# jwliao1209/DiffMusic

Hardware: AMD Instinct MI355X
Metric: denoising steps/sec (10 s clip, 200-step DPS) (higher is better)
Workload: dtype f16; 1 GPU; MusicLDM + DPS music_inpainting, 10 s @16 kHz, 200-step schedule, batch 8 per GPU (BASELINE.json configs[1]); global_batch=8, clips_per_gpu=8, lanes=1, parallelism=clip-sharded x1 (RCCL world size 1, no per-step collective), finite=True, nan_steps=0, settle_steps=10, cached_reference_transform=True, launched_by=single process

## Files before the change

### diffmusic_amd/_lib.py

```python
import ctypes as C
import os

_HERE = os.path.dirname(os.path.abspath(__file__))
LIB_PATH = os.environ.get("DMX_LIB_PATH") or os.path.join(_HERE, "lib", "libdiffmusic_hip.so")
MAX_STAGES = 8


class HifiGanConfig(C.Structure):
    _fields_ = [("model_in_dim", C.c_int), ("upsample_initial_channel", C.c_int), ("num_upsamples", C.c_int),
                ("upsample_rates", C.c_int * MAX_STAGES), ("upsample_kernel_sizes", C.c_int * MAX_STAGES),
                ("num_kernels", C.c_int), ("resblock_kernel_sizes", C.c_int * MAX_STAGES),
                ("num_dilations", C.c_int), ("resblock_dilation_sizes", C.c_int * (MAX_STAGES * MAX_STAGES)),
                ("leaky_relu_slope", C.c_float)]


class VaeConfig(C.Structure):
    _fields_ = [("latent_channels", C.c_int), ("out_channels", C.c_int), ("num_blocks", C.c_int),
                ("block_out_channels", C.c_int * MAX_STAGES), ("layers_per_block", C.c_int),
                ("norm_num_groups", C.c_int), ("eps", C.c_float)]


class UNetConfig(C.Structure):
    _fields_ = [("in_channels", C.c_int), ("out_channels", C.c_int), ("num_blocks", C.c_int),
                ("block_out_channels", C.c_int * MAX_STAGES), ("layers_per_block", C.c_int),
# ... 65 lines not shown
    "dmx_vae_encode_fwd": (C.c_int, [C.c_void_p, C.c_void_p, C.c_float, C.c_void_p, C.c_int, C.c_int, C.c_int, C.c_void_p, C.c_size_t,
                                     C.c_void_p]),
    "dmx_latent_init": (C.c_int, [C.c_void_p] * 6 + [C.c_int] * 3 + [C.c_float] * 3 + [C.c_void_p]),
    "dmx_conv2d_raw": (C.c_int, [C.c_void_p] * 4 + [C.c_int] * 9 + [C.c_void_p]),
    "dmx_unet_workspace_bytes": (C.c_size_t, [C.c_void_p, C.c_int, C.c_int, C.c_int]),
    "dmx_unet_fwd": (C.c_int, [C.c_void_p, C.c_void_p, C.c_void_p, C.c_void_p, C.c_void_p, C.c_int, C.c_int, C.c_int,
                               C.c_void_p, C.c_size_t, C.c_void_p]),
    "dmx_unet_fwd_ctx": (C.c_int, [C.c_void_p] * 5 + [C.c_int, C.c_void_p, C.c_int, C.c_void_p, C.c_void_p, C.c_int, C.c_int, C.c_int,
                                   C.c_void_p, C.c_size_t, C.c_void_p]),
    "dmx_unet_workspace_bytes_ctx": (C.c_size_t, [C.c_void_p, C.c_int, C.c_int, C.c_int, C.c_int, C.c_int]),
    "dmx_htsat_create": (C.c_void_p, [C.POINTER(HtsatConfig)]),
    "dmx_htsat_feature_dims": (C.c_int, [C.c_void_p, C.POINTER(C.c_int), C.POINTER(C.c_int)]),
    "dmx_htsat_workspace_bytes": (C.c_size_t, [C.c_void_p, C.c_int, C.c_int]),
    "dmx_htsat_fwd": (C.c_int, [C.c_void_p, C.c_void_p, C.c_int, C.c_int, C.c_void_p, C.c_int, C.c_void_p, C.c_size_t, C.c_void_p]),
    "dmx_htsat_bwd": (C.c_int, [C.c_void_p, C.c_void_p, C.c_void_p, C.c_void_p, C.c_void_p]),
    "dmx_htsat_tape_raw": (C.c_size_t, [C.c_void_p, C.c_int, C.c_int, C.c_int, C.c_void_p, C.c_size_t, C.c_void_p]),
    "dmx_gram_fwd": (C.c_int, [C.c_void_p, C.c_void_p, C.c_int, C.c_int, C.c_int, C.c_void_p]),
    "dmx_gram_bwd": (C.c_int, [C.c_void_p, C.c_void_p, C.c_void_p, C.c_int, C.c_int, C.c_int, C.c_void_p]),
    "dmx_gemm_raw": (C.c_int, [C.c_void_p, C.c_size_t, C.c_void_p]),
    "dmx_prof_begin": (None, []),
    "dmx_prof_end": (C.c_int, [C.POINTER(C.c_double), C.POINTER(C.c_double)]),
    "dmx_flash_attn_raw": (C.c_int, [C.c_void_p, C.c_void_p, C.c_void_p, C.c_void_p, C.c_void_p] + [C.c_int] * 6 + [C.c_float, C.c_void_p]),
    "dmx_flash_attn_ld_raw": (C.c_int, [C.c_void_p] * 5 + [C.c_int] * 8 + [C.c_float, C.POINTER(C.c_int), C.c_void_p]),
    "dmx_softmax_raw": (C.c_int, [C.c_void_p] * 3 + [C.c_longlong, C.c_int, C.c_longlong, C.c_longlong, C.c_int, C.c_void_p]),
    "dmx_softmax_act_raw": (C.c_int, [C.c_void_p] * 3 + [C.c_longlong, C.c_int, C.c_longlong, C.c_int, C.c_void_p]),
    "dmx_transpose_raw": (C.c_int, [C.c_void_p, C.c_void_p, C.c_int, C.c_int, C.c_longlong, C.c_longlong, C.c_int, C.c_int] + [C.c_longlong] * 4
                          + [C.c_void_p]),
    "dmx_rowdot_raw": (C.c_int, [C.c_void_p] * 3 + [C.c_longlong, C.c_int, C.c_longlong, C.c_longlong, C.c_void_p]),
    "dmx_layernorm_raw": (C.c_int, [C.c_void_p] * 4 + [C.c_int, C.c_int, C.c_float, C.c_void_p]),
    "dmx_geglu_raw": (C.c_int, [C.c_void_p, C.c_void_p, C.c_longlong, C.c_int, C.c_void_p]),
    "dmx_gemm_splitk_workspace": (C.c_int, [C.c_void_p, C.c_size_t]),
    "dmx_conv_pair_raw": (C.c_int, [C.c_void_p, C.c_void_p, C.c_size_t, C.c_void_p]),
    "dmx_conv_pair_group_raw": (C.c_int, [C.c_int, C.c_void_p, C.c_void_p, C.c_size_t, C.c_void_p]),
    "dmx_groupnorm_scratch_floats": (C.c_size_t, [C.c_int, C.c_int, C.c_int]),
    "dmx_groupnorm_raw": (C.c_int, [C.c_void_p] * 8 + [C.c_int] * 4 + [C.c_float, C.c_int, C.c_void_p]),
    "dmx_groupnorm_part_floats": (C.c_size_t, [C.c_int, C.c_int, C.c_int]),
    "dmx_groupnorm_parts_raw": (C.c_int, [C.c_void_p] * 7 + [C.c_int] * 4 + [C.c_float, C.c_int, C.c_int, C.c_void_p, C.c_void_p, C.c_void_p]),
    "dmx_gemm_last_tile_rows_raw": (C.c_int, []),
    "dmx_groupnorm_bwd_raw": (C.c_int, [C.c_void_p] * 10 + [C.c_int] * 6 + [C.c_void_p, C.c_void_p, C.c_void_p]),
    "dmx_prof_dominant": (C.c_int, [C.POINTER(C.c_double)] * 3),
    "dmx_audio_create": (C.c_void_p, [C.c_int, C.c_int, C.c_int, C.c_int, C.c_void_p]),
    "dmx_audio_destroy": (None, [C.c_void_p]),
    "dmx_audio_num_frames": (C.c_int, [C.c_void_p, C.c_int]),
    "dmx_audio_num_bins": (C.c_int, [C.c_void_p]),
    "dmx_audio_state_bytes": (C.c_size_t, [C.c_void_p, C.c_int, C.c_int]),
    "dmx_audio_transform_fwd": (C.c_int, [C.c_void_p, C.c_void_p, C.c_longlong, C.c_void_p, C.c_void_p, C.c_int, C.c_int, C.c_int,
                                          C.c_int, C.c_float, C.c_float, C.c_void_p]),
    "dmx_audio_transform_bwd": (C.c_int, [C.c_void_p, C.c_void_p, C.c_void_p, C.c_longlong, C.c_void_p, C.c_int, C.c_int, C.c_int,
                                          C.c_int, C.c_float, C.c_float, C.c_int, C.c_void_p]),
    "dmx_audio_is_fused": (C.c_int, [C.c_void_p, C.c_int]),
    "dmx_audio_guidance_fwd": (C.c_int, [C.c_void_p, C.c_void_p, C.c_longlong, C.c_void_p, C.c_void_p, C.c_longlong, C.c_void_p, C.c_void_p,
                                         C.c_int, C.c_int, C.c_int, C.c_int, C.c_float, C.c_float, C.c_void_p]),
    "dmx_audio_guidance_bwd": (C.c_int, [C.c_void_p, C.c_void_p, C.c_longlong, C.c_void_p, C.c_void_p, C.c_longlong, C.c_float, C.c_void_p,
                                         C.c_void_p, C.c_longlong, C.c_int, C.c_void_p, C.c_int, C.c_int, C.c_int, C.c_int, C.c_float, C.c_float,
                                         C.c_void_p]),
    "dmx_audio_guidance_fwd_ex": (C.c_int, [C.c_void_p, C.c_void_p, C.c_longlong, C.c_void_p, C.c_void_p, C.c_longlong, C.c_void_p, C.c_void_p,
                                            C.c_int, C.c_int, C.c_int, C.c_int, C.c_float, C.c_float, C.c_void_p, C.c_longlong, C.c_void_p,
                                            C.c_float, C.c_void_p]),
    "dmx_audio_guidance_bwd_ex": (C.c_int, [C.c_void_p, C.c_void_p, C.c_longlong, C.c_void_p, C.c_void_p, C.c_longlong, C.c_float, C.c_void_p,
                                            C.c_void_p, C.c_longlong, C.c_int, C.c_void_p, C.c_int, C.c_int, C.c_int, C.c_int, C.c_float, C.c_float,
                                            C.c_void_p, C.c_longlong, C.c_void_p, C.c_float, C.c_void_p]),
    "dmx_audio_guidance_fwd_shaped": (C.c_int, [C.c_void_p, C.c_void_p, C.c_longlong, C.c_void_p, C.c_void_p, C.c_longlong, C.c_void_p, C.c_void_p,
                                                C.c_int, C.c_int, C.c_int, C.c_int, C.c_float, C.c_float, C.c_void_p, C.c_longlong, C.c_void_p,
                                                C.c_float, C.c_void_p, C.c_void_p]),
    "dmx_audio_guidance_bwd_shaped": (C.c_int, [C.c_void_p, C.c_void_p, C.c_longlong, C.c_void_p, C.c_void_p, C.c_longlong, C.c_float, C.c_void_p,
                                                C.c_void_p, C.c_longlong, C.c_int, C.c_void_p, C.c_int, C.c_int, C.c_int, C.c_int, C.c_float, C.c_float,
# ... 86 lines not shown
```

### diffmusic_amd/csrc/capi.hip

```cpp
#include "conv_pair.h"
#include "models.h"

#define M_IMPL(m) ((m) ? (m)->impl : nullptr)
#define ST(s) ((hipStream_t)(s))

extern "C" {

int dmx_abi_version(void) { return DMX_ABI_VERSION; }
int dmx_act_dtype(void) { return DMX_ACT_DTYPE; }

dmx_model* dmx_hifigan_create(const dmx_hifigan_config* cfg) {
  if (!cfg || cfg->num_upsamples > DMX_MAX_STAGES || cfg->num_kernels > DMX_MAX_STAGES || cfg->num_dilations > DMX_MAX_STAGES) {
    dmx_set_error("bad hifigan config");
    return nullptr;
  }
  return new dmx_model{dmx_make_hifigan(cfg)};
}
dmx_model* dmx_vae_decoder_create(const dmx_vae_config* cfg) {
  if (!cfg || cfg->num_blocks > DMX_MAX_STAGES) { dmx_set_error("bad vae config"); return nullptr; }
  Model* m = dmx_make_vae(cfg);
  return m ? new dmx_model{m} : nullptr;
}
dmx_model* dmx_unet_create(const dmx_unet_config* cfg) {
  if (!cfg || cfg->num_blocks > DMX_MAX_STAGES) { dmx_set_error("bad unet config"); return nullptr; }
// ... 138 lines not shown
}

size_t dmx_unet_workspace_bytes(dmx_model* m, int batch, int h, int w) { return dmx_unet_ws_impl(m->impl, batch, h, w, 0, 0); }
size_t dmx_unet_workspace_bytes_ctx(dmx_model* m, int batch, int h, int w, int n0, int n1) { return dmx_unet_ws_impl(m->impl, batch, h, w, n0, n1); }
int dmx_unet_fwd(dmx_model* m, const float* x, const float* t, const float* class_labels, float* eps, int batch, int h, int w,
                 void* ws, size_t ws_bytes, void* stream) {
  int rc = check(m, DMX_MODEL_UNET);
  if (rc) return rc;
  if (!ws) { dmx_set_error("null workspace"); return DMX_ERR_WORKSPACE; }
  return dmx_unet_fwd_impl(m->impl, x, t, class_labels, eps, batch, h, w, ws, ws_bytes, ST(stream), nullptr, 0, nullptr, 0, nullptr);
}
int dmx_unet_fwd_ctx(dmx_model* m, const float* x, const float* t, const float* class_labels, const float* ctx0, int n0,
                     const float* ctx1, int n1, const float* bias1, float* eps, int batch, int h, int w, void* ws, size_t ws_bytes,
                     void* stream) {
  int rc = check(m, DMX_MODEL_UNET);
  if (rc) return rc;
  if (!ws) { dmx_set_error("null workspace"); return DMX_ERR_WORKSPACE; }
  return dmx_unet_fwd_impl(m->impl, x, t, class_labels, eps, batch, h, w, ws, ws_bytes, ST(stream), ctx0, n0, ctx1, n1, bias1);
}

static thread_local int g_raw_gn_rows = 0;
int dmx_gemm_raw(const void* desc, size_t desc_bytes, void* stream) {
  if (desc_bytes != sizeof(GemmDesc)) { dmx_set_error("GemmDesc size mismatch: %zu vs %zu", desc_bytes, sizeof(GemmDesc)); return DMX_ERR_SHAPE; }
  return dmx_gemm_launch(*reinterpret_cast<const GemmDesc*>(desc), ST(stream), &g_raw_gn_rows);
}
int dmx_gemm_last_tile_rows_raw(void) { return g_raw_gn_rows; }

int dmx_conv_pair_raw(const void* desc_a, const void* desc_b, size_t desc_bytes, void* stream) {
  if (desc_bytes != sizeof(GemmDesc)) { dmx_set_error("GemmDesc size mismatch: %zu vs %zu", desc_bytes, sizeof(GemmDesc)); return DMX_ERR_SHAPE; }
  const GemmDesc* a = reinterpret_cast<const GemmDesc*>(desc_a);
  const GemmDesc& b = *reinterpret_cast<const GemmDesc*>(desc_b);
  if (!dmx_conv_pair_eligible(a, b)) { dmx_set_error("shape not handled by the fused convolution-pair kernel"); return DMX_ERR_SHAPE; }
  return dmx_conv_pair_launch(a, b, ST(stream));
}

int dmx_conv_pair_group_raw(int n, const void* descs_a, const void* descs_b, size_t desc_bytes, void* stream) {
  if (desc_bytes != sizeof(GemmDesc)) { dmx_set_error("GemmDesc size mismatch: %zu vs %zu", desc_bytes, sizeof(GemmDesc)); return DMX_ERR_SHAPE; }
  if (n < 1 || n > 3) { dmx_set_error("conv pair group: 1..3 problems"); return DMX_ERR_SHAPE; }
  const GemmDesc* a = reinterpret_cast<const GemmDesc*>(descs_a);
  const GemmDesc* b = reinterpret_cast<const GemmDesc*>(descs_b);
  const GemmDesc* pa[3]; const GemmDesc* pb[3];
  for (int j = 0; j < n; ++j) { pa[j] = a + j; pb[j] = b + j; }
  const int rc = dmx_conv_pair_group_launch(n, pa, pb, ST(stream));
  if (rc == DMX_ERR_SHAPE) dmx_set_error("shape not handled by the fused convolution-pair kernel");
  return rc;
}

int dmx_flash_attn_raw(const void* q, const void* k, const void* v, void* o, const float* colbias, int B, int Nq, int Nk, int ldv, int C,
                       int heads, float scale, void* stream) {
  const int rc = dmx_flash_attn_fwd((const act_t*)q, (const act_t*)k, (const act_t*)v, (act_t*)o, colbias, B, Nq, Nk, C, heads, scale,
                                    ST(stream), 0, 0, ldv);
  if (rc == DMX_ERR_SHAPE) dmx_set_error("flash attention: unsupported head_dim / strides");
  return rc;
}

int dmx_flash_attn_ld_raw(const void* q, const void* k, const void* v, void* o, const float* colbias, int B, int Nq, int Nk, int ldq, int ldk,
                          int ldv, int C, int heads, float scale, int* qt_out, void* stream) {
  if (qt_out) *qt_out = 0;
  if (B < 1 || heads < 1 || C < heads || C % heads) { dmx_set_error("flash attention: C %d is not heads %d x head_dim", C, heads); return DMX_ERR_SHAPE; }
  const int rc = dmx_flash_attn_fwd((const act_t*)q, (const act_t*)k, (const act_t*)v, (act_t*)o, colbias, B, Nq, Nk, C, heads, scale,
                                    ST(stream), ldq, ldk, ldv, qt_out);
  if (rc == DMX_ERR_SHAPE)
    dmx_set_error("flash attention: head_dim %d (multiples of 8 up to 96), Nq %d, Nk %d (>= 1) or row strides %d / %d / %d (multiples of 8) unsupported",
                  C / heads, Nq, Nk, ldq, ldk, ldv);
  return rc;
}
// ... 85 lines not shown
```

### diffmusic_amd/csrc/conv_pair.hip

```cpp
#include "gemm_epilogue.h"
#include "conv_pair.h"

namespace {

constexpr int PAIR_HALO = 50;
constexpr int PAIR_ROWS = 256;
constexpr unsigned PAIR_OOB = 0x80000000u;

struct PairParams {
  GemmDesc a, b;
  int T, nb, BMo;
  int loA, hiA, loB, hiB;
  int off0A, dA, off0B, dB;
  int single;
  int r_from_slab;
  int a_tape_bits_only;
  int skip_q0, skip_n;
  int z0, z1;
};

#ifdef DMX_PAIR_STAMPS
__device__ unsigned long long g_pair_stamps[4096 * 8];
#define DMX_STAMP(i) do { stamp_v[i] = wall_clock64(); } while (0)
#else
#define DMX_STAMP(i) do { } while (0)
#endif

template <int C>
struct PairCfg {
  static constexpr int PITCH = 2 * C + 32;
  static constexpr int CPR = C / 8;
  static constexpr int WN = C > 64 ? C / 64 : 1;
  static constexpr int NW = 4 * WN;
  static constexpr int NT = NW * 64;
  static constexpr int FN = C / 16 / WN;
  static constexpr int SLAB_ROWS = PAIR_ROWS + PAIR_HALO;
  static constexpr int SLAB_BYTES = SLAB_ROWS * PITCH;
  static constexpr int TILE = C * 128;
  static constexpr int NS = C == 128 ? 4 : 3;
  static constexpr int PER = TILE / 1024 / NW;
  static constexpr int SLAB_IT = (SLAB_ROWS * CPR + NT - 1) / NT;
  static constexpr int BITS_IT = PAIR_ROWS * CPR / NT;
  static constexpr int BITS_BYTES = PAIR_ROWS * CPR;
  static constexpr int BIAS_BYTES = 2 * C * 4;
  static constexpr int LDS_BYTES = SLAB_BYTES + NS * TILE + BITS_BYTES + BIAS_BYTES;
  static constexpr int MIN_WAVES = C == 32 ? 3 : 2;
  static_assert(PER >= 1 && PAIR_ROWS * CPR % NT == 0, "tile / thread-count mismatch");
};

template <int FN>
struct PairFrags { frag8_t x[2][4]; frag8_t w[2][FN]; };

#define DMX_PAIR_DSR(dst, addr, off) asm volatile("ds_read_b128 %0, %1 offset:%2" : "=v"(dst) : "v"(addr), "n"(off))

#define DMX_LDS_ADDR(p) ((unsigned)(size_t)(__attribute__((address_space(3))) const char*)(p))
typedef unsigned u32x2_t __attribute__((ext_vector_type(2)));
typedef unsigned u32x4_t __attribute__((ext_vector_type(4)));
__device__ __forceinline__ void pair_lds_w64(const void* p, uint2 v) {
// ... 8 lines not shown
  asm volatile("s_waitcnt lgkmcnt(0)" : "+v"(r[0]), "+v"(r[1]), "+v"(r[2]), "+v"(r[3]), "+v"(r[4]), "+v"(r[5]), "+v"(r[6]), "+v"(r[7]) : : "memory");
}
template <typename T>
__device__ __forceinline__ void pair_tie16(T (&r)[16]) {
  asm volatile("s_waitcnt lgkmcnt(0)"
               : "+v"(r[0]), "+v"(r[1]), "+v"(r[2]), "+v"(r[3]), "+v"(r[4]), "+v"(r[5]), "+v"(r[6]), "+v"(r[7]), "+v"(r[8]), "+v"(r[9]), "+v"(r[10]),
                 "+v"(r[11]), "+v"(r[12]), "+v"(r[13]), "+v"(r[14]), "+v"(r[15])
               :
               : "memory");
}
template <typename T, int N>
__device__ __forceinline__ void pair_tie(T (&r)[N]) {
  static_assert(N == 8 || N == 16, "4 row fragments x 2 or 4 column fragments");
  if constexpr (N == 8) pair_tie8(r); else pair_tie16(r);
}

__device__ __forceinline__ void pair_settle(PairFrags<4>& f) {
  asm volatile("s_waitcnt lgkmcnt(0)"
               : "+v"(f.x[0][0]), "+v"(f.x[0][1]), "+v"(f.x[0][2]), "+v"(f.x[0][3]), "+v"(f.x[1][0]), "+v"(f.x[1][1]), "+v"(f.x[1][2]),
                 "+v"(f.x[1][3]), "+v"(f.w[0][0]), "+v"(f.w[0][1]), "+v"(f.w[0][2]), "+v"(f.w[0][3]), "+v"(f.w[1][0]), "+v"(f.w[1][1]),
                 "+v"(f.w[1][2]), "+v"(f.w[1][3])
               :
               : "memory");
}
__device__ __forceinline__ void pair_settle(PairFrags<2>& f) {
  asm volatile("s_waitcnt lgkmcnt(0)"
               : "+v"(f.x[0][0]), "+v"(f.x[0][1]), "+v"(f.x[0][2]), "+v"(f.x[0][3]), "+v"(f.x[1][0]), "+v"(f.x[1][1]), "+v"(f.x[1][2]),
                 "+v"(f.x[1][3]), "+v"(f.w[0][0]), "+v"(f.w[0][1]), "+v"(f.w[1][0]), "+v"(f.w[1][1])
               :
               : "memory");
}

template <int C>
__device__ __forceinline__ void pair_body(const PairParams& P, char* smem, int bid, const int nwg) {
  using K = PairCfg<C>;
  constexpr int PITCH = K::PITCH, CPR = K::CPR, FN = K::FN, NS = K::NS, PER = K::PER, TILE = K::TILE, NT = K::NT, NW = K::NW, WN = K::WN;
  char* ring = smem;
  char* slab = smem + NS * TILE;
  unsigned char* s_bits = reinterpret_cast<unsigned char*>(slab + K::SLAB_BYTES);
  float* s_bias = reinterpret_cast<float*>(slab + K::SLAB_BYTES + K::BITS_BYTES);

  const int tid = threadIdx.x, lane = tid & 63, lr = lane & 15, lq = lane >> 4;
  const int wave = __builtin_amdgcn_readfirstlane(tid >> 6);
  const int rg = wave / WN, cg = wave - rg * WN;
#ifdef DMX_PAIR_STAMPS
  const int stamp_id = bid;
  unsigned long long stamp_v[8] = {0, 0, 0, 0, 0, 0, 0, 0};
#endif
  DMX_STAMP(0);
  {
    const int q = nwg >> 3, r = nwg & 7, xcd = bid & 7, loc = bid >> 3;
    bid = (xcd < r ? xcd * (q + 1) : r * (q + 1) + (xcd - r) * q) + loc;
  }
  const int T = P.T;
  const int b = bid / P.nb;
  int tq = bid - b * P.nb;
  if (tq >= P.skip_q0) tq += P.skip_n;
  const int t0 = tq * P.BMo;
  const bool single = P.single != 0;
  const int kA = single ? 0 : P.a.ntaps, kB = P.b.ntaps;
  const int stepsA = (kA * C + 63) / 64, stepsB = (kB * C + 63) / 64, total = stepsA + stepsB;

  const __amdgpu_buffer_rsrc_t rsA = __builtin_amdgcn_make_buffer_rsrc(const_cast<act_t*>(single ? P.b.W : P.a.W), 0, PAIR_OOB, 0x00020000);
  const __amdgpu_buffer_rsrc_t rsB = __builtin_amdgcn_make_buffer_rsrc(const_cast<act_t*>(P.b.W), 0, PAIR_OOB, 0x00020000);
  const int lrow = lane >> 3, cc = (lane & 7) ^ lrow;
  auto issue_dma = [&](int g) {
    const bool inA = g < stepsA;
    const int sidx = inA ? g : g - stepsA;
    const int Kel = inA ? P.a.K : P.b.K;
    const unsigned ldw2 = (unsigned)(inA ? P.a.ldw : P.b.ldw) * 2u;
    const int kel = sidx * 64 + cc * 8;
    const bool ok = g < total && kel < Kel;
    char* dst = ring + (g % NS) * TILE;
#pragma unroll
    for (int i = 0; i < PER; ++i) {
      const int j = i * NW + wave;
      const unsigned voff = ok ? (unsigned)(j * 8 + lrow) * ldw2 + (unsigned)kel * 2u : PAIR_OOB;
      if (inA) __builtin_amdgcn_raw_ptr_buffer_load_lds(rsA, (__attribute__((address_space(3))) void*)(dst + j * 1024), 16, voff, 0, 0, 0);
      else __builtin_amdgcn_raw_ptr_buffer_load_lds(rsB, (__attribute__((address_space(3))) void*)(dst + j * 1024), 16, voff, 0, 0, 0);
    }
  };
  issue_dma(0);
  issue_dma(1);
  issue_dma(2);

  {
    const act_t* src = single ? P.b.A : P.a.A;
    const int nrows = PAIR_ROWS + (single ? P.loB + P.hiB : P.loA + P.hiA);
    const int tfirst = t0 - P.loB - (single ? 0 : P.loA);
    uint4 sv[K::SLAB_IT];
#pragma unroll
    for (int it = 0; it < K::SLAB_IT; ++it) {
      const int c = tid + it * NT, row = c / CPR, piece = c % CPR, t = tfirst + row;
      sv[it] = make_uint4(0, 0, 0, 0);
      if (row < nrows && t >= 0 && t < T && !(t >= P.z0 && t < P.z1)) sv[it] = *reinterpret_cast<const uint4*>(src + ((long long)b * T + t) * C + piece * 8);
    }
    const bool masked = !single && (P.a.flags & EPI_MASK);
    const bool maskbits = !single && (P.a.flags & EPI_MASKBITS);
    constexpr int BPT = K::BITS_BYTES / NT;
    static_assert(BPT == 4 || BPT == 8, "bit-mask copy granularity");
    static_assert(CPR % BPT == 0, "a thread's mask bytes must stay inside one row");
    uint32_t mb[2] = {0u, 0u};
    if (maskbits) {
      const int c = tid * BPT, row = c / CPR, piece = c % CPR, t = t0 - P.loB + row;
      if (t >= 0 && t < T) {
        const unsigned char* src = P.a.XB + ((long long)b * T + t) * P.a.ldxb + piece;
        mb[0] = *reinterpret_cast<const uint32_t*>(src);
        if (BPT == 8) mb[1] = *reinterpret_cast<const uint32_t*>(src + 4);
      }
    }
#pragma unroll
    for (int it = 0; it < K::SLAB_IT; ++it) {
      const int c = tid + it * NT, row = c / CPR, piece = c % CPR;
      if (row < K::SLAB_ROWS) *reinterpret_cast<uint4*>(slab + row * PITCH + piece * 16) = sv[it];
    }
    if (masked) {
#pragma unroll 1
      for (int it = 0; it < K::BITS_IT; ++it) {
        const int c = tid + it * NT, row = c / CPR, piece = c % CPR, t = t0 - P.loB + row;
        uint4 m = make_uint4(0, 0, 0, 0);
        if (t >= 0 && t < T) m = *reinterpret_cast<const uint4*>(P.a.X + ((long long)b * T + t) * C + piece * 8);
        s_bits[c] = (unsigned char)dmx_pos8(m);
      }
    }
    if (maskbits) {
      uint32_t* d = reinterpret_cast<uint32_t*>(s_bits + tid * BPT);
      d[0] = mb[0];
      if (BPT == 8) d[1] = mb[1];
    }
  }
  if (tid < 2 * C) {
    const GemmDesc& d = tid < C ? P.a : P.b;
    const int ch = tid < C ? tid : tid - C;
    s_bias[tid] = (!(single && tid < C) && d.bias && (d.flags & (EPI_BIAS | EPI_BIASINIT))) ? d.bias[ch] : 0.f;
  }
  asm volatile("s_waitcnt vmcnt(0)" ::: "memory");
  __syncthreads();
  DMX_STAMP(1);

  f32x4 acc[4][FN];
  auto zero_acc = [&]() {
#pragma unroll
    for (int i = 0; i < 4; ++i)
#pragma unroll
      for (int n = 0; n < FN; ++n) acc[i][n] = f32x4{0.f, 0.f, 0.f, 0.f};
  };
  auto init_acc = [&](const GemmDesc& d) {
    if (C < 128 && (d.flags & EPI_BIASINIT)) {
      f32x4 bb[FN];
#pragma unroll
      for (int n = 0; n < FN; ++n)
        asm volatile("ds_read_b128 %0, %1" : "=v"(bb[n]) : "v"(DMX_LDS_ADDR(s_bias + (&d == &P.b ? C : 0) + cg * 64 + n * 16 + lq * 4)));
      if constexpr (FN == 2) asm volatile("s_waitcnt lgkmcnt(0)" : "+v"(bb[0]), "+v"(bb[1]) : : "memory");
      else asm volatile("s_waitcnt lgkmcnt(0)" : "+v"(bb[0]), "+v"(bb[1]), "+v"(bb[2]), "+v"(bb[3]) : : "memory");
#pragma unroll
      for (int n = 0; n < FN; ++n)
#pragma unroll
        for (int i = 0; i < 4; ++i) acc[i][n] = bb[n];
    } else {
      zero_acc();
    }
  };
  using Frags = PairFrags<FN>;
  const unsigned xlane = (unsigned)(size_t)(__attribute__((address_space(3))) const char*)(slab + (rg * 64 + lr) * PITCH + lq * 16);
  const unsigned wlane0 = (unsigned)(size_t)(__attribute__((address_space(3))) const char*)(ring + (cg * 64 + lr) * 128 + (((0 * 4 + lq) ^ (lr & 7)) << 4));
  const unsigned wlane1 = (unsigned)(size_t)(__attribute__((address_space(3))) const char*)(ring + (cg * 64 + lr) * 128 + (((1 * 4 + lq) ^ (lr & 7)) << 4));
  auto load_frags = [&](Frags& f, bool isB, int sidx, int g) {
    const int off0 = isB ? P.off0B : P.off0A, dd = isB ? P.dB : P.dA, kk = isB ? kB : kA;
    unsigned xa0, xa1;
    if constexpr (C >= 64) {
      constexpr int SPT = C / 64;
// ... 157 lines not shown
      u32x4_t tq[K::BITS_IT];
#pragma unroll
      for (int it = 0; it < K::BITS_IT; ++it) {
        const int c = tid + it * NT, row = c / CPR, piece = c % CPR;
        asm volatile("ds_read_b128 %0, %1" : "=v"(tq[it]) : "v"(DMX_LDS_ADDR(slab + row * PITCH + piece * 16)));
      }
      static_assert(K::BITS_IT == 4 || K::BITS_IT == 8, "tape read-back granularity");
      if constexpr (K::BITS_IT == 4)
        asm volatile("s_waitcnt lgkmcnt(0)" : "+v"(tq[0]), "+v"(tq[1]), "+v"(tq[2]), "+v"(tq[3]) : : "memory");
      else
        asm volatile("s_waitcnt lgkmcnt(0)" : "+v"(tq[0]), "+v"(tq[1]), "+v"(tq[2]), "+v"(tq[3]), "+v"(tq[4]), "+v"(tq[5]), "+v"(tq[6]), "+v"(tq[7]) : : "memory");
      uint4 tv[K::BITS_IT];
#pragma unroll
      for (int it = 0; it < K::BITS_IT; ++it) tv[it] = make_uint4(tq[it][0], tq[it][1], tq[it][2], tq[it][3]);
#pragma unroll
      for (int it = 0; it < K::BITS_IT; ++it) {
        const int c = tid + it * NT, row = c / CPR, piece = c % CPR, t = t0 - P.loB + row;
        if (row >= P.loB && row < P.loB + P.BMo && t < T) {
          if (full) *reinterpret_cast<uint4*>(P.a.C2 + ((long long)b * T + t) * C + piece * 8) = tv[it];
        }
        if constexpr (C < 128) {
          if (bits) tape_bits[it >> 2] |= (dmx_pos8(tv[it]) & 0xffu) << (8 * (it & 3));
        } else {
          if (bits && row >= P.loB && row < P.loB + P.BMo && t < T) P.a.B2[((long long)b * T + t) * P.a.ldb2 + piece] = (unsigned char)dmx_pos8(tv[it]);
        }
      }
      tape_bits_valid = bits && C < 128;
    }
  }

  DMX_STAMP(3);
  init_acc(P.b);
  run_stage(true, stepsB, stepsA);
  __syncthreads();
  DMX_STAMP(4);
  {
    constexpr int EPI_WAVE_BYTES = 64 * (FN * 32 + 16) + 64 * 12;
    static_assert(EPI_WAVE_BYTES * NW <= K::SLAB_BYTES, "epilogue staging does not fit the slab");
    const int mbase = b * T + t0;
    const int tend = t0 + P.BMo < T ? t0 + P.BMo : T;
    gemm_epilogue_lds_impl<4, FN, 1>(P.b, acc, mbase + rg * 64, cg * 64, lane, 0, T, slab + wave * EPI_WAVE_BYTES, b * T + tend, rpre,
                                        !single && P.r_from_slab != 0);
  }
  if (tape_bits_valid) {
#pragma unroll
    for (int it = 0; it < K::BITS_IT; ++it) {
      const int c = tid + it * NT, row = c / CPR, piece = c % CPR, t = t0 - P.loB + row;
      if (row >= P.loB && row < P.loB + P.BMo && t < T)
        P.a.B2[((long long)b * T + t) * P.a.ldb2 + piece] = (unsigned char)((tape_bits[it >> 2] >> (8 * (it & 3))) & 0xffu);
    }
  }
  DMX_STAMP(5);
#ifdef DMX_PAIR_STAMPS
  if (threadIdx.x == 0 && stamp_id < 4096)
    for (int i = 0; i < 8; ++i) g_pair_stamps[stamp_id * 8 + i] = stamp_v[i];
#endif
}

template <int C>
__global__ __launch_bounds__(PairCfg<C>::NT, PairCfg<C>::MIN_WAVES) void conv_pair_kernel(const PairParams P) {
  extern __shared__ __attribute__((aligned(1024))) char smem[];
  pair_body<C>(P, smem, blockIdx.x, gridDim.x);
}

constexpr int DMX_PAIR_GROUP = 3;
struct PairGroup { PairParams p[DMX_PAIR_GROUP]; int n[DMX_PAIR_GROUP]; };
template <int C>
__global__ __launch_bounds__(PairCfg<C>::NT, PairCfg<C>::MIN_WAVES) void conv_pair_group_kernel(const PairGroup G) {
  extern __shared__ __attribute__((aligned(1024))) char smem[];
  const int j = blockIdx.y, n = G.n[j];
  if ((int)blockIdx.x >= n) return;
  pair_body<C>(G.p[j], smem, blockIdx.x, n);
}

struct Halo { int lo, hi; bool ok; int d; };
Halo halo_of(const GemmDesc& d) {
  Halo h{0, 0, true, d.ntaps > 1 ? d.tdx[1] - d.tdx[0] : 0};
  for (int j = 0; j < d.ntaps; ++j) {
    if (d.tdx[j] != d.tdx[0] + j * h.d) h.ok = false;
    if (d.tdy[j] != 0) h.ok = false;
    if (-d.tdx[j] > h.lo) h.lo = -d.tdx[j];
    if (d.tdx[j] > h.hi) h.hi = d.tdx[j];
  }
  if (h.lo + h.hi > PAIR_HALO) h.ok = false;
  return h;
}

bool stage_ok(const GemmDesc& d, int C, int T, int allowed_flags) {
  if (d.N != C || d.Ci != C || d.lda != C || d.K != d.ntaps * C || d.ldw < d.K) return false;
  if (d.ntaps < 1 || d.ntaps > 16 || d.Z != 1 || d.Hq != 1 || d.Hi != 1 || d.Ho != 1) return false;
  if (d.Wq != T || d.Wi != T || d.Wo != T || d.sx != 1 || d.osx != 1 || d.oox != 0 || d.ooy != 0) return false;
  if (d.flags & ~allowed_flags) return false;
  if (d.M % T != 0) return false;
  return true;
}

bool g_pair_enabled = getenv("DMX_NO_PAIR") == nullptr;

}

bool dmx_conv_pair_eligible(const GemmDesc* a, const GemmDesc& b) {
  if (!g_pair_enabled) return false;
  const int C = b.N, T = b.Wq;
  static const bool c128 = getenv("DMX_NO_PAIR128") == nullptr;
  if (C != 32 && C != 64 && !(C == 128 && c128)) return false;
// ... 45 lines not shown
  {
    int q0, q1;
    pair_skip_slabs(dead, P.T, P.BMo, q0, q1);
    P.skip_q0 = q0; P.skip_n = q1 - q0;
    P.nb -= P.skip_n;
    if (dead && dead->zero1 > dead->zero0) { P.z0 = dead->zero0; P.z1 = dead->zero1; }
  }
  static const bool bias_init = getenv("DMX_NO_BIAS_INIT") == nullptr;
  if (bias_init && b.N < 128) {
    if ((P.b.flags & EPI_BIAS) && P.b.bias && !(P.b.flags & (EPI_MASK | EPI_MASKBITS))) P.b.flags = (P.b.flags & ~EPI_BIAS) | EPI_BIASINIT;
    if (a && (P.a.flags & EPI_BIAS) && P.a.bias && !(P.a.flags & (EPI_MASK | EPI_MASKBITS))) P.a.flags = (P.a.flags & ~EPI_BIAS) | EPI_BIASINIT;
  }
  P.r_from_slab = (a && (b.flags & EPI_RESID) && b.R == a->A && b.ldr == b.N) ? 1 : 0;
  P.a_tape_bits_only = (a && (a->flags & EPI_BITS2) && !a->C2) ? 1 : 0;
  const int nclips = b.M / P.T;
  const int C = b.N;
  fl = 2.0 * b.M * (double)b.N * b.K;
  by = 2.0 * b.M * (double)C * 2.0;
  const double bits_by = b.M * (double)C / 8.0;
  if (a) {
    fl += 2.0 * a->M * (double)a->N * a->K;
    if ((a->flags & EPI_LRELU2) && !P.a_tape_bits_only) by += 2.0 * b.M * (double)C;
    if (a->flags & EPI_BITS2) by += bits_by;
    if (a->flags & EPI_MASK) by += 2.0 * b.M * (double)C;
    if (a->flags & EPI_MASKBITS) by += bits_by;
  }
  if ((b.flags & EPI_RESID) && !P.r_from_slab) by += 2.0 * b.M * (double)C;
  if (b.flags & EPI_MASK) by += 2.0 * b.M * (double)C;
  if (b.flags & EPI_MASKBITS) by += bits_by;
  if (b.flags & EPI_BITS2) by += bits_by;
  if (b.flags & EPI_ACCUM) by += 2.0 * b.M * (double)C;
  if ((b.flags & EPI_LRELU2) && !(b.flags & EPI_NO_C)) by += 2.0 * b.M * (double)C;
  fl *= (double)P.nb / nb_all; by *= (double)P.nb / nb_all;
  return (long long)nclips * P.nb;
}
bool pair_zero_ok(const PairParams& P) { return P.z1 <= P.z0 || !(P.b.flags & EPI_RESID) || P.r_from_slab; }
}

void dmx_conv_pair_slabs(const GemmDesc* a, const GemmDesc& b, const PairDead* dead, int* skipped, int* total) {
  const Halo hb = halo_of(b);
  const int T = b.Wq, BMo = a ? PAIR_ROWS - hb.lo - hb.hi : PAIR_ROWS;
  int q0, q1;
  pair_skip_slabs(dead, T, BMo, q0, q1);
  *skipped = q1 - q0;
  *total = cdiv(T, BMo);
}

static int pair_extra_lds() { static const int v = [] { const char* e = getenv("DMX_PAIR_EXTRA_LDS"); return e ? atoi(e) : 0; }(); return v; }
int dmx_conv_pair_launch(const GemmDesc* a, const GemmDesc& b, hipStream_t st, const PairDead* dead) {
  if (!dmx_conv_pair_eligible(a, b)) return DMX_ERR_SHAPE;
  PairParams P;
  double fl, by;
  const long long grid = pair_params(a, b, P, fl, by, dead);
  if (grid > 0x7fffffffLL) return DMX_ERR_SHAPE;
  if (!pair_zero_ok(P)) return DMX_ERR_SHAPE;
  const int C = b.N;
  const int rec = dmx_prof_open(st);
  auto launch = [&](auto tag) {
    constexpr int CC = decltype(tag)::value;
    static bool attr = false;
    if (!attr) { (void)hipFuncSetAttribute((const void*)conv_pair_kernel<CC>, hipFuncAttributeMaxDynamicSharedMemorySize, PairCfg<CC>::LDS_BYTES + (CC < 128 ? pair_extra_lds() : 0)); attr = true; }
    hipLaunchKernelGGL(conv_pair_kernel<CC>, dim3((unsigned)grid), dim3(PairCfg<CC>::NT), PairCfg<CC>::LDS_BYTES + (CC < 128 ? pair_extra_lds() : 0), st, P);
  };
  if (C == 32) launch(std::integral_constant<int, 32>{});
  else if (C == 64) launch(std::integral_constant<int, 64>{});
  else launch(std::integral_constant<int, 128>{});
  dmx_prof_close(rec, st, fl, by, b.M, b.N, (a ? a->K : 0) + b.K, b.ntaps, b.flags, a ? 21 : 20);
  return hipGetLastError() == hipSuccess ? DMX_OK : DMX_ERR_LAUNCH;
}

int dmx_conv_pair_group_launch(int n, const GemmDesc* const* a, const GemmDesc* const* b, hipStream_t st, const PairDead* dead) {
  if (n < 1 || n > DMX_PAIR_GROUP) return DMX_ERR_SHAPE;
  static const bool off = getenv("DMX_NO_PAIR_GROUP") != nullptr;
  bool same = !off && n > 1;
  for (int j = 0; j < n; ++j) {
    if (!a[j] || !b[j] || !dmx_conv_pair_eligible(a[j], *b[j])) return DMX_ERR_SHAPE;
    if (b[j]->N != b[0]->N) same = false;
    for (int i = 0; i < j; ++i)
      if (b[j]->C == b[i]->C || (b[j]->C2 && b[j]->C2 == b[i]->C2)) same = false;
  }
  if (!same) {
    for (int j = 0; j < n; ++j) { const int rc = dmx_conv_pair_launch(a[j], *b[j], st, dead ? dead + j : nullptr); if (rc != DMX_OK) return rc; }
    return DMX_OK;
  }
  int order[DMX_PAIR_GROUP] = {0, 1, 2};
  auto work = [&](int j) { return a[j]->K + b[j]->K; };
  for (int i = 0; i < n; ++i)
    for (int k = i + 1; k < n; ++k)
      if (work(order[k]) > work(order[i])) { const int t = order[i]; order[i] = order[k]; order[k] = t; }
  PairGroup G;
  memset(&G, 0, sizeof(G));
  double fl = 0.0, by = 0.0;
  long long gmax = 0;
  int Ksum = 0;
  for (int i = 0; i < n; ++i) {
    const int j = order[i];
    double f1, b1;
    const long long g = pair_params(a[j], *b[j], G.p[i], f1, b1, dead ? dead + j : nullptr);
    if (g > 0x7ffffff0LL || !pair_zero_ok(G.p[i])) return DMX_ERR_SHAPE;
    G.n[i] = (int)g;
    if (g > gmax) gmax = g;
    fl += f1; by += b1; Ksum += a[j]->K + b[j]->K;
  }
  const unsigned gx = (unsigned)((gmax + 7) & ~7ll);
  const int C = b[0]->N;
  const int rec = dmx_prof_open(st);
  auto launch = [&](auto tag) {
    constexpr int CC = decltype(tag)::value;
    static bool attr = false;
    if (!attr) { (void)hipFuncSetAttribute((const void*)conv_pair_group_kernel<CC>, hipFuncAttributeMaxDynamicSharedMemorySize, PairCfg<CC>::LDS_BYTES); attr = true; }
    hipLaunchKernelGGL(conv_pair_group_kernel<CC>, dim3(gx, (unsigned)n), dim3(PairCfg<CC>::NT), PairCfg<CC>::LDS_BYTES, st, G);
  };
  if (C == 32) launch(std::integral_constant<int, 32>{});
  else if (C == 64) launch(std::integral_constant<int, 64>{});
  else launch(std::integral_constant<int, 128>{});
  dmx_prof_close(rec, st, fl, by, b[0]->M, C, Ksum, b[0]->ntaps, b[0]->flags, 22);
  return hipGetLastError() == hipSuccess ? DMX_OK : DMX_ERR_LAUNCH;
}

#ifdef DMX_PAIR_STAMPS
extern "C" int dmx_pair_stamps_read(unsigned long long* host) {
  return hipMemcpyFromSymbol(host, HIP_SYMBOL(g_pair_stamps), sizeof(unsigned long long) * 4096 * 8) == hipSuccess ? 0 : -1;
}
#endif
```

### include/diffmusic_hip.h

```cpp
#ifndef DIFFMUSIC_HIP_H
#define DIFFMUSIC_HIP_H
#include <stddef.h>
#include <stdint.h>

#ifdef __cplusplus
extern "C" {
#endif

#define DMX_ABI_VERSION 4
#define DMX_MAX_STAGES 8

typedef struct dmx_model dmx_model;

typedef struct dmx_hifigan_config {
  int model_in_dim;
  int upsample_initial_channel;
  int num_upsamples;
  int upsample_rates[DMX_MAX_STAGES];
  int upsample_kernel_sizes[DMX_MAX_STAGES];
  int num_kernels;
  int resblock_kernel_sizes[DMX_MAX_STAGES];
  int num_dilations;
  int resblock_dilation_sizes[DMX_MAX_STAGES * DMX_MAX_STAGES];
  float leaky_relu_slope;
// ... 166 lines not shown
int dmx_sched_pred_x0(const float* x, const float* eps, float* x0, long long n, float alpha_t, void* stream);
int dmx_sched_pred_x0_ex(const float* x, const float* model_output, float* x0, long long n, float alpha_t, int prediction_type, float clip_range,
                         void* stream);
int dmx_sched_cfg_combine(const float* eps2, float* out, long long n, float scale, void* stream);
int dmx_sched_step(int mode, const float* x, const float* eps, const float* x0, const float* g0, const float* inv_scale,
                   const float* noise, float* prev, float* x0_out, float* grad_out, int batch, int n, float alpha_t, float alpha_prev,
                   float sigma, float rate, float eps_small, int global_norm, void* stream);
int dmx_sched_step_ex(int mode, const float* x, const float* eps, const float* x0, const float* g0, const float* inv_scale,
                      const float* noise, float* prev, float* x0_out, float* grad_out, int batch, int n, float alpha_t, float alpha_prev,
                      float sigma, float rate, float eps_small, int global_norm, int prediction_type, float clip_range, void* stream);

int dmx_randn_philox(float* out, int batch, long long n, const unsigned long long* seeds_host, unsigned long long offset, void* stream);

void dmx_prof_begin(void);
int dmx_prof_end(double* total_ms, double* total_flops);
int dmx_prof_dominant(double* ms, double* flops, double* bytes);

int dmx_gemm_raw(const void* desc, size_t desc_bytes, void* stream);
int dmx_flash_attn_raw(const void* q, const void* k, const void* v, void* o, const float* colbias, int B, int Nq, int Nk, int ldv,
                       int C, int heads, float scale, void* stream);
int dmx_flash_attn_ld_raw(const void* q, const void* k, const void* v, void* o, const float* colbias, int B, int Nq, int Nk, int ldq,
                          int ldk, int ldv, int C, int heads, float scale, int* qt_out, void* stream);
int dmx_softmax_raw(const float* S, void* P, const float* colbias, long long rows, int N, long long lds, long long ldp, int rows_per_bias,
                    void* stream);
int dmx_softmax_act_raw(const void* S, void* P, const float* colbias, long long rows, int N, long long ldp, int rows_per_bias, void* stream);
int dmx_transpose_raw(const void* in, void* out, int R, int C, long long ldi, long long ldo, int Z, int Zi, long long sIo, long long sIi,
                      long long sOo, long long sOi, void* stream);
int dmx_rowdot_raw(const void* a, const void* b, float* out, long long rows, int C, long long lda, long long ldb, void* stream);
int dmx_layernorm_raw(const void* x, void* y, const float* gamma, const float* beta, int rows, int C, float eps, void* stream);
int dmx_geglu_raw(const void* x, void* y, long long rows, int I, void* stream);
int dmx_gemm_splitk_workspace(void* ws, size_t bytes);
int dmx_conv_pair_raw(const void* desc_a, const void* desc_b, size_t desc_bytes, void* stream);
int dmx_conv_pair_group_raw(int n, const void* descs_a, const void* descs_b, size_t desc_bytes, void* stream);
size_t dmx_groupnorm_scratch_floats(int B, int C, int G);
int dmx_groupnorm_raw(const void* x, void* y, const float* gamma, const float* beta, float* stats, float* scale, float* shift,
                      float* partial, int B, int P, int C, int G, float eps, int silu, void* stream);
size_t dmx_groupnorm_part_floats(int B, int P, int N);
int dmx_groupnorm_parts_raw(const void* x, void* y, const float* gamma, const float* beta, float* stats, float* scale, float* shift,
                            int B, int P, int C, int G, float eps, int silu, int nreg, float* const* part, const int* geom, void* stream);
int dmx_gemm_last_tile_rows_raw(void);
int dmx_conv2d_raw(const float* w_host, const float* b_host, const void* x, void* y, int B, int Hi, int Wi, int Ci, int Co, int k, int stride,
                   int pad_lo, int pad_hi, void* stream);
int dmx_groupnorm_bwd_raw(const void* x, const void* dy, const void* add, void* dx, const float* stats, const float* scale, const float* shift,
                          float* k0, float* k1, float* partial, int B, int P, int C, int G, int silu, int nreg, float* const* part,
                          const int* geom, void* stream);

#ifdef __cplusplus
}
#endif
#endif
```

Baseline: 26.45 steps/s (weak scaling: one step advances a batch of 8 clips on one GPU; value = K / wall x 1 GPU(s)).

## Make fused conv-pair kernels persistent with grid-stride loops capped at residency

```diff
diff --git a/diffmusic_amd/_lib.py b/diffmusic_amd/_lib.py
--- a/diffmusic_amd/_lib.py
+++ b/diffmusic_amd/_lib.py
@@ -121,6 +121,7 @@
     "dmx_gemm_splitk_workspace": (C.c_int, [C.c_void_p, C.c_size_t]),
     "dmx_conv_pair_raw": (C.c_int, [C.c_void_p, C.c_void_p, C.c_size_t, C.c_void_p]),
     "dmx_conv_pair_group_raw": (C.c_int, [C.c_int, C.c_void_p, C.c_void_p, C.c_size_t, C.c_void_p]),
+    "dmx_conv_pair_dead_raw": (C.c_int, [C.c_void_p, C.c_void_p, C.c_size_t, C.c_int, C.c_int, C.c_int, C.c_int, C.c_void_p]),
     "dmx_groupnorm_scratch_floats": (C.c_size_t, [C.c_int, C.c_int, C.c_int]),
     "dmx_groupnorm_raw": (C.c_int, [C.c_void_p] * 8 + [C.c_int] * 4 + [C.c_float, C.c_int, C.c_void_p]),
     "dmx_groupnorm_part_floats": (C.c_size_t, [C.c_int, C.c_int, C.c_int]),
diff --git a/diffmusic_amd/csrc/capi.hip b/diffmusic_amd/csrc/capi.hip
--- a/diffmusic_amd/csrc/capi.hip
+++ b/diffmusic_amd/csrc/capi.hip
@@ -194,6 +194,18 @@
   const GemmDesc& b = *reinterpret_cast<const GemmDesc*>(desc_b);
   if (!dmx_conv_pair_eligible(a, b)) { dmx_set_error("shape not handled by the fused convolution-pair kernel"); return DMX_ERR_SHAPE; }
   return dmx_conv_pair_launch(a, b, ST(stream));
+}
+
+int dmx_conv_pair_dead_raw(const void* desc_a, const void* desc_b, size_t desc_bytes, int skip0, int skip1, int zero0, int zero1,
+                           void* stream) {
+  if (desc_bytes != sizeof(GemmDesc)) { dmx_set_error("GemmDesc size mismatch: %zu vs %zu", desc_bytes, sizeof(GemmDesc)); return DMX_ERR_SHAPE; }
+  const GemmDesc* a = reinterpret_cast<const GemmDesc*>(desc_a);
+  const GemmDesc& b = *reinterpret_cast<const GemmDesc*>(desc_b);
+  if (!dmx_conv_pair_eligible(a, b)) { dmx_set_error("shape not handled by the fused convolution-pair kernel"); return DMX_ERR_SHAPE; }
+  PairDead pd; pd.skip0 = skip0; pd.skip1 = skip1; pd.zero0 = zero0; pd.zero1 = zero1;
+  const int rc = dmx_conv_pair_launch(a, b, ST(stream), &pd);
+  if (rc == DMX_ERR_SHAPE) dmx_set_error("conv pair: rows read as zeros need the second stage's residual to be the first stage's input");
+  return rc;
 }
 
 int dmx_conv_pair_group_raw(int n, const void* descs_a, const void* descs_b, size_t desc_bytes, void* stream) {
diff --git a/diffmusic_amd/csrc/conv_pair.hip b/diffmusic_amd/csrc/conv_pair.hip
--- a/diffmusic_amd/csrc/conv_pair.hip
+++ b/diffmusic_amd/csrc/conv_pair.hip
@@ -17,13 +17,17 @@
   int a_tape_bits_only;
   int skip_q0, skip_n;
   int z0, z1;
+  int nitems;
 };
 
 #ifdef DMX_PAIR_STAMPS
 __device__ unsigned long long g_pair_stamps[4096 * 8];
+int g_pair_stamp_rows = 0;
+#define DMX_STAMP_ROWS(n) do { g_pair_stamp_rows = (n) < 4096 ? (int)(n) : 4096; } while (0)
 #define DMX_STAMP(i) do { stamp_v[i] = wall_clock64(); } while (0)
 #else
 #define DMX_STAMP(i) do { } while (0)
+#define DMX_STAMP_ROWS(n) do { } while (0)
 #endif
 
 template <int C>
@@ -98,7 +102,7 @@
 }
 
 template <int C>
-__device__ __forceinline__ void pair_body(const PairParams& P, char* smem, int bid, const int nwg) {
+__device__ __forceinline__ void pair_body(const PairParams& P, char* smem, int bid, const int nwg, const bool again, const int stamp_row) {
   using K = PairCfg<C>;
   constexpr int PITCH = K::PITCH, CPR = K::CPR, FN = K::FN, NS = K::NS, PER = K::PER, TILE = K::TILE, NT = K::NT, NW = K::NW, WN = K::WN;
   char* ring = smem;
@@ -106,11 +110,13 @@
   unsigned char* s_bits = reinterpret_cast<unsigned char*>(slab + K::SLAB_BYTES);
   float* s_bias = reinterpret_cast<float*>(slab + K::SLAB_BYTES + K::BITS_BYTES);
 
-  const int tid = threadIdx.x, lane = tid & 63, lr = lane & 15, lq = lane >> 4;
+  int tid = threadIdx.x;
+  asm volatile("" : "+v"(tid));
+  const int lane = tid & 63, lr = lane & 15, lq = lane >> 4;
   const int wave = __builtin_amdgcn_readfirstlane(tid >> 6);
   const int rg = wave / WN, cg = wave - rg * WN;
 #ifdef DMX_PAIR_STAMPS
-  const int stamp_id = bid;
+  const int stamp_id = stamp_row;
   unsigned long long stamp_v[8] = {0, 0, 0, 0, 0, 0, 0, 0};
 #endif
   DMX_STAMP(0);
@@ -175,6 +181,7 @@
         if (BPT == 8) mb[1] = *reinterpret_cast<const uint32_t*>(src + 4);
       }
     }
+    if (again) __builtin_amdgcn_s_barrier();
 #pragma unroll
     for (int it = 0; it < K::SLAB_IT; ++it) {
       const int c = tid + it * NT, row = c / CPR, piece = c % CPR;
@@ -203,6 +210,7 @@
   asm volatile("s_waitcnt vmcnt(0)" ::: "memory");
   __syncthreads();
   DMX_STAMP(1);
+  asm volatile("" : "+v"(tid));
 
   f32x4 acc[4][FN];
   auto zero_acc = [&]() {
@@ -426,6 +434,7 @@
   DMX_STAMP(3);
   init_acc(P.b);
   run_stage(true, stepsB, stepsA);
+  asm volatile("s_waitcnt vmcnt(0)" ::: "memory");
   __syncthreads();
   DMX_STAMP(4);
   {
@@ -446,25 +455,44 @@
   }
   DMX_STAMP(5);
 #ifdef DMX_PAIR_STAMPS
-  if (threadIdx.x == 0 && stamp_id < 4096)
+  if (threadIdx.x == 0 && stamp_id >= 0 && stamp_id < 4096)
     for (int i = 0; i < 8; ++i) g_pair_stamps[stamp_id * 8 + i] = stamp_v[i];
 #endif
 }
 
+template <typename T>
+__device__ __forceinline__ const T& pair_kernarg() {
+  auto p = __builtin_amdgcn_kernarg_segment_ptr();
+  asm volatile("" : "+s"(p));
+  return *(const T*)p;
+}
 template <int C>
-__global__ __launch_bounds__(PairCfg<C>::NT, PairCfg<C>::MIN_WAVES) void conv_pair_kernel(const PairParams P) {
+__global__ __launch_bounds__(PairCfg<C>::NT, PairCfg<C>::MIN_WAVES) void conv_pair_kernel(const PairParams) {
   extern __shared__ __attribute__((aligned(1024))) char smem[];
-  pair_body<C>(P, smem, blockIdx.x, gridDim.x);
+  const int w = blockIdx.x, step = gridDim.x;
+  for (int item = w;; item += step) {
+    const PairParams& P = pair_kernarg<PairParams>();
+    if (item >= P.nitems) break;
+    pair_body<C>(P, smem, item, P.nitems, item != w, item);
+  }
 }
 
 constexpr int DMX_PAIR_GROUP = 3;
-struct PairGroup { PairParams p[DMX_PAIR_GROUP]; int n[DMX_PAIR_GROUP]; };
+struct PairGroup { PairParams p[DMX_PAIR_GROUP]; int start[DMX_PAIR_GROUP]; int nitems; };
 template <int C>
-__global__ __launch_bounds__(PairCfg<C>::NT, PairCfg<C>::MIN_WAVES) void conv_pair_group_kernel(const PairGroup G) {
+__global__ __launch_bounds__(PairCfg<C>::NT, PairCfg<C>::MIN_WAVES) void conv_pair_group_kernel(const PairGroup) {
   extern __shared__ __attribute__((aligned(1024))) char smem[];
-  const int j = blockIdx.y, n = G.n[j];
-  if ((int)blockIdx.x >= n) return;
-  pair_body<C>(G.p[j], smem, blockIdx.x, n);
+  const int w = blockIdx.x, step = gridDim.x;
+  bool again = false;
+  for (int item = w;; item += step) {
+    const PairGroup& G = pair_kernarg<PairGroup>();
+    if (item >= G.nitems) break;
+    const int j = (item >= G.start[1] ? 1 : 0) + (item >= G.start[2] ? 1 : 0);
+    const int loc = item - G.start[j], n = G.p[j].nitems;
+    if (loc >= n) continue;
+    pair_body<C>(G.p[j], smem, loc, n, again, item);
+    again = true;
+  }
 }
 
 struct Halo { int lo, hi; bool ok; int d; };
@@ -576,7 +604,9 @@
   if (b.flags & EPI_ACCUM) by += 2.0 * b.M * (double)C;
   if ((b.flags & EPI_LRELU2) && !(b.flags & EPI_NO_C)) by += 2.0 * b.M * (double)C;
   fl *= (double)P.nb / nb_all; by *= (double)P.nb / nb_all;
-  return (long long)nclips * P.nb;
+  const long long items = (long long)nclips * P.nb;
+  P.nitems = items > 0x7fffffffLL ? 0 : (int)items;
+  return items;
 }
 bool pair_zero_ok(const PairParams& P) { return P.z1 <= P.z0 || !(P.b.flags & EPI_RESID) || P.r_from_slab; }
 }
@@ -588,6 +618,26 @@
   pair_skip_slabs(dead, T, BMo, q0, q1);
   *skipped = q1 - q0;
   *total = cdiv(T, BMo);
+}
+
+namespace {
+int pair_resident(const void* fn, int threads, int lds) {
+  (void)hipFuncSetAttribute(fn, hipFuncAttributeMaxDynamicSharedMemorySize, lds);
+  int dev = 0, per = 0;
+  hipDeviceProp_t prop;
+  if (hipGetDevice(&dev) != hipSuccess || hipGetDeviceProperties(&prop, dev) != hipSuccess) return 0;
+  if (hipOccupancyMaxActiveBlocksPerMultiprocessor(&per, fn, threads, (size_t)lds) != hipSuccess || per < 1) return 0;
+  return per * prop.multiProcessorCount;
+}
+bool pair_loops_by_default(int C, bool grouped) { return !grouped && (C == 64 || C == 128); }
+unsigned pair_grid(long long items, int resident, int C, bool grouped) {
+  const char* e = getenv("DMX_PAIR_GRID_CAP");
+  long long cap = e ? atoll(e) : 0;
+  if (cap == 0) cap = pair_loops_by_default(C, grouped) && resident > 0 ? resident : -1;
+  if (cap < 0) return (unsigned)items;
+  cap = (cap + 7) & ~7ll;
+  return (unsigned)(items < cap ? items : cap);
+}
 }
 
 static int pair_extra_lds() { static const int v = [] { const char* e = getenv("DMX_PAIR_EXTRA_LDS"); return e ? atoi(e) : 0; }(); return v; }
@@ -599,12 +649,13 @@
   if (grid > 0x7fffffffLL) return DMX_ERR_SHAPE;
   if (!pair_zero_ok(P)) return DMX_ERR_SHAPE;
   const int C = b.N;
+  DMX_STAMP_ROWS(grid);
   const int rec = dmx_prof_open(st);
   auto launch = [&](auto tag) {
     constexpr int CC = decltype(tag)::value;
-    static bool attr = false;
-    if (!attr) { (void)hipFuncSetAttribute((const void*)conv_pair_kernel<CC>, hipFuncAttributeMaxDynamicSharedMemorySize, PairCfg<CC>::LDS_BYTES + (CC < 128 ? pair_extra_lds() : 0)); attr = true; }
-    hipLaunchKernelGGL(conv_pair_kernel<CC>, dim3((unsigned)grid), dim3(PairCfg<CC>::NT), PairCfg<CC>::LDS_BYTES + (CC < 128 ? pair_extra_lds() : 0), st, P);
+    const int lds = PairCfg<CC>::LDS_BYTES + (CC < 128 ? pair_extra_lds() : 0);
+    static const int resident = pair_resident((const void*)conv_pair_kernel<CC>, PairCfg<CC>::NT, lds);
+    hipLaunchKernelGGL(conv_pair_kernel<CC>, dim3(pair_grid(grid, resident, CC, false)), dim3(PairCfg<CC>::NT), lds, st, P);
   };
   if (C == 32) launch(std::integral_constant<int, 32>{});
   else if (C == 64) launch(std::integral_constant<int, 64>{});
@@ -635,25 +686,27 @@
   PairGroup G;
   memset(&G, 0, sizeof(G));
   double fl = 0.0, by = 0.0;
-  long long gmax = 0;
+  long long items = 0;
   int Ksum = 0;
+  for (int i = 0; i < DMX_PAIR_GROUP; ++i) G.start[i] = 0x7fffffff;
   for (int i = 0; i < n; ++i) {
     const int j = order[i];
     double f1, b1;
     const long long g = pair_params(a[j], *b[j], G.p[i], f1, b1, dead ? dead + j : nullptr);
     if (g > 0x7ffffff0LL || !pair_zero_ok(G.p[i])) return DMX_ERR_SHAPE;
-    G.n[i] = (int)g;
-    if (g > gmax) gmax = g;
+    G.start[i] = (int)items;
+    items += (g + 7) & ~7ll;
+    if (items > 0x7ffffff0LL) return DMX_ERR_SHAPE;
     fl += f1; by += b1; Ksum += a[j]->K + b[j]->K;
   }
-  const unsigned gx = (unsigned)((gmax + 7) & ~7ll);
+  G.nitems = (int)items;
+  DMX_STAMP_ROWS(items);
   const int C = b[0]->N;
   const int rec = dmx_prof_open(st);
   auto launch = [&](auto tag) {
     constexpr int CC = decltype(tag)::value;
-    static bool attr = false;
-    if (!attr) { (void)hipFuncSetAttribute((const void*)conv_pair_group_kernel<CC>, hipFuncAttributeMaxDynamicSharedMemorySize, PairCfg<CC>::LDS_BYTES); attr = true; }
-    hipLaunchKernelGGL(conv_pair_group_kernel<CC>, dim3(gx, (unsigned)n), dim3(PairCfg<CC>::NT), PairCfg<CC>::LDS_BYTES, st, G);
+    static const int resident = pair_resident((const void*)conv_pair_group_kernel<CC>, PairCfg<CC>::NT, PairCfg<CC>::LDS_BYTES);
+    hipLaunchKernelGGL(conv_pair_group_kernel<CC>, dim3(pair_grid(items, resident, CC, true)), dim3(PairCfg<CC>::NT), PairCfg<CC>::LDS_BYTES, st, G);
   };
   if (C == 32) launch(std::integral_constant<int, 32>{});
   else if (C == 64) launch(std::integral_constant<int, 64>{});
@@ -664,6 +717,6 @@
 
 #ifdef DMX_PAIR_STAMPS
 extern "C" int dmx_pair_stamps_read(unsigned long long* host) {
-  return hipMemcpyFromSymbol(host, HIP_SYMBOL(g_pair_stamps), sizeof(unsigned long long) * 4096 * 8) == hipSuccess ? 0 : -1;
+  return hipMemcpyFromSymbol(host, HIP_SYMBOL(g_pair_stamps), sizeof(unsigned long long) * 4096 * 8) == hipSuccess ? g_pair_stamp_rows : -1;
 }
 #endif
diff --git a/include/diffmusic_hip.h b/include/diffmusic_hip.h
--- a/include/diffmusic_hip.h
+++ b/include/diffmusic_hip.h
@@ -222,6 +222,8 @@
 int dmx_gemm_splitk_workspace(void* ws, size_t bytes);
 int dmx_conv_pair_raw(const void* desc_a, const void* desc_b, size_t desc_bytes, void* stream);
 int dmx_conv_pair_group_raw(int n, const void* descs_a, const void* descs_b, size_t desc_bytes, void* stream);
+int dmx_conv_pair_dead_raw(const void* desc_a, const void* desc_b, size_t desc_bytes, int skip0, int skip1, int zero0, int zero1,
+                           void* stream);
 size_t dmx_groupnorm_scratch_floats(int B, int C, int G);
 int dmx_groupnorm_raw(const void* x, void* y, const float* gamma, const float* beta, float* stats, float* scale, float* shift,
                       float* partial, int B, int P, int C, int G, float eps, int silu, void* stream);
```

Result: no change. 26.38 steps/s (weak scaling: one step advances a batch of 8 clips on one GPU; value = K / wall x 1 GPU(s)) (-0.3%).
